# rust-seq/simd-minimizers

Hardware: AMD Instinct MI355X
Metric: Gbases/s (whole node) for canonical minimizers k=21 w=11 on 3.1 Gbp; HBM GB/s %peak (higher is better)
Workload: dtype u32

## Files before the change

### include/simd_minimizers_amd.h

```cpp
#ifndef SIMD_MINIMIZERS_AMD_H
#define SIMD_MINIMIZERS_AMD_H

#include <stddef.h>
#include <stdint.h>

#ifdef __cplusplus
extern "C" {
#endif


typedef struct mm_hasher {
    uint32_t fw[4];
    uint32_t rc[4];
    uint32_t rot;
    uint32_t canonical;
    uint32_t fw_xor;
    uint32_t rc_xor;
    uint32_t kind;
} mm_hasher_t;

typedef enum mm_hasher_kind { MM_HASHER_NT = 0, MM_HASHER_MUL = 1, MM_HASHER_ANTILEX = 2 } mm_hasher_kind_t;

typedef enum mm_mode { MM_MINIMIZERS = 0, MM_CLOSED_SYNCMERS = 1, MM_OPEN_SYNCMERS = 2 } mm_mode_t;

// ... 252 lines not shown

int mm_device_group_upload_batch(mm_device_group_t *group, uint64_t n_seqs, const uint8_t *const *packed,
                                 const uint64_t *packed_bytes);
int mm_run_batch_sharded_device(const mm_plan_t *plan, mm_device_group_t *group, const uint64_t *base_offsets ,
                                const uint64_t *n_bases, int want_superkmers, uint64_t *out_counts ,
                                uint64_t *total);
int mm_device_group_batch_result(const mm_device_group_t *group, uint64_t seq, int *entry, uint32_t **d_pos,
                                 uint32_t **d_sk, uint64_t *count);
int mm_device_group_gather_batch(mm_device_group_t *group, int root, uint32_t *d_dst_pos, uint32_t *d_dst_sk ,
                                 uint64_t capacity, uint64_t *out_offsets );

int mm_debug_launch_plan(uint32_t w, int canonical_windows, int mode, uint64_t n_seqs, const uint64_t *n_windows,
                         uint64_t *out7, uint32_t *tile_seq, uint32_t *tile_win0, uint32_t *tile_nblk,
                         uint64_t tile_capacity, uint64_t *n_tiles);
int mm_debug_launch_lds(uint32_t w, int canonical_windows, int mode, uint64_t n_windows, uint64_t *out2);
int mm_debug_lane_plan(uint32_t k, uint32_t w, int canonical_windows, int mode, uint64_t n_reads, uint64_t total_bases,
                       uint32_t blocks_per_lane, uint64_t *out6);
int mm_debug_last_lane_table(mm_workspace_t *ws, uint32_t *out4, uint64_t capacity, uint64_t *n_lanes);
int mm_link_probe(mm_workspace_t *ws, const void *host_in, void *host_out, uint64_t bytes, double *out_GBps );
int mm_clock_probe_begin(mm_workspace_t *ws, uint64_t duration_us);
int mm_clock_probe_end(mm_workspace_t *ws, double *ghz);
int mm_generate_device_async(mm_workspace_t *ws, uint64_t seed, uint64_t first_base,
                             uint64_t n_bases, uint8_t *d_packed );

#ifdef __cplusplus
}
#endif
#endif
```

### simd-minimizers_amd/__init__.py

```python
from __future__ import annotations

import ctypes as C
import os
import threading

import numpy as np

_HERE = os.path.dirname(os.path.abspath(__file__))
LIB_PATH = os.environ.get("MM_LIB_PATH") or os.path.join(_HERE, "libsimd_minimizers_amd.so")

MM_MINIMIZERS, MM_CLOSED_SYNCMERS, MM_OPEN_SYNCMERS = 0, 1, 2
PATH_FUSED, PATH_GENERIC, PATH_SPLIT = 1, 2, 3
U64_MAX = (1 << 64) - 1

ERR = {
    "W_ZERO": -1, "W_TOO_LARGE": -2, "LEN_TOO_LARGE": -3, "EVEN_L": -4,
    "HASHER_NOT_CANONICAL": -5, "OPEN_EVEN_W": -6, "K_ZERO": -7, "CAPACITY": -8, "BAD_MODE": -9,
    "NULL": -10, "VALUE_LEN": -11, "FORMAT": -12, "NO_DEVICE": -20, "HIP": -21, "ALLOC": -22, "ORDER": -23,
    "UNSORTED": -24,
}


class MinimizerError(RuntimeError):
    def __init__(self, code: int, msg: str):
# ... 118 lines not shown
            L.mm_device_group_upload_batch.argtypes = [vp, C.c_uint64, C.POINTER(u8p), u64p]
            L.mm_run_batch_sharded_device.argtypes = [vp, vp, u64p, u64p, C.c_int, u64p, u64p]
            L.mm_device_group_batch_result.argtypes = [vp, C.c_uint64, C.POINTER(C.c_int), C.POINTER(u32p), C.POINTER(u32p), u64p]
            L.mm_device_group_gather_batch.argtypes = [vp, C.c_int, vp, vp, C.c_uint64, u64p]
            L.mm_run_packed_reads_device_async.argtypes = [vp, vp, vp, C.c_uint64, C.c_uint64, C.c_uint64, vp, C.c_uint64,
                                                           C.c_uint32, vp, vp, C.c_uint64, vp, vp]
            L.mm_run_packed_reads_device.argtypes = [vp, vp, vp, C.c_uint64, C.c_uint64, C.c_uint64, vp, C.c_uint64,
                                                     C.c_uint32, vp, vp, C.c_uint64, vp, u64p]
            L.mm_run_packed_reads_host.argtypes = [vp, vp, u8p, C.c_uint64, u64p, C.c_uint32, u32p, u32p, C.c_uint64, u64p, u64p]
            L.mm_debug_launch_plan.argtypes = [C.c_uint32, C.c_int, C.c_int, C.c_uint64, u64p, u64p, u32p, u32p, u32p,
                                               C.c_uint64, u64p]
        L.mm_clock_probe_begin.argtypes = [vp, C.c_uint64]
        L.mm_clock_probe_end.argtypes = [vp, C.POINTER(C.c_double)]
        L.mm_link_probe.argtypes = [vp, vp, vp, C.c_uint64, C.POINTER(C.c_double)]
        L.mm_debug_launch_lds.argtypes = [C.c_uint32, C.c_int, C.c_int, C.c_uint64, u64p]
        L.mm_debug_lane_plan.argtypes = [C.c_uint32, C.c_uint32, C.c_int, C.c_int, C.c_uint64, C.c_uint64, C.c_uint32, u64p]
        L.mm_debug_last_lane_table.argtypes = [vp, u32p, C.c_uint64, u64p]
        L.mm_fused_overread_bytes.argtypes = []
        L.mm_fused_overread_bytes.restype = C.c_uint64
        L.mm_workspace_force_generic.argtypes = [vp, C.c_int]
        L.mm_workspace_set_blocks_per_lane.argtypes = [vp, C.c_uint32]
        L.mm_workspace_enable_timing.argtypes = [vp, C.c_int]
        L.mm_workspace_kernel_time.argtypes = [vp, C.POINTER(C.c_double), u64p, C.c_int]
        L.mm_workspace_last_path.argtypes = [vp]
        L.mm_workspace_ticket_mode.argtypes = [vp]
        L.mm_workspace_last_lane_table.argtypes = [vp]
        if hasattr(L, "mm_prebuilt_window_sizes"):
            L.mm_prebuilt_window_sizes.argtypes = [C.c_int, C.c_int, u32p, C.c_int]
            L.mm_prebuilt_window_sizes.restype = C.c_int
        L.mm_run_device_async.argtypes = [vp, vp, vp, C.c_uint64, C.c_uint64, C.c_uint64, C.c_uint64,
# ... 70 lines not shown
    "mm_run_device_async", "mm_run_device", "mm_run_host", "mm_run_host_ascii",
    "mm_values_u64_device_async", "mm_values_u64_host", "mm_values_u128_device_async",
    "mm_values_u128_host", "mm_run_batch_device", "mm_run_reads_device_async", "mm_run_reads_device",
    "mm_run_reads_superkmers_device_async", "mm_run_reads_superkmers_device",
    "mm_run_skip_ambiguous_device_async", "mm_run_skip_ambiguous_device", "mm_run_skip_ambiguous_host",
    "mm_run_skip_ambiguous_host_ascii", "mm_run_reads_skip_ambiguous_device_async",
    "mm_run_reads_skip_ambiguous_device", "mm_pack_ascii_n_device_async", "mm_pack_ascii_device_async",
    "mm_host_alloc", "mm_host_free",
    "mm_generate_device_async", "mm_fasta_pack_device_async", "mm_fasta_pack_device", "mm_fastq_pack_device_async",
    "mm_clock_probe_begin", "mm_clock_probe_end", "mm_link_probe", "mm_fused_overread_bytes",
    "mm_device_group_create", "mm_device_group_destroy", "mm_device_group_size", "mm_run_sharded_host",
    "mm_run_batch_sharded_host",
    "mm_device_group_upload", "mm_device_group_upload_range", "mm_device_group_adopt", "mm_run_sharded_device", "mm_device_group_result",
    "mm_device_group_gather",
    "mm_device_group_upload_batch", "mm_run_batch_sharded_device", "mm_device_group_batch_result",
    "mm_device_group_gather_batch", "mm_debug_launch_plan", "mm_debug_launch_lds", "mm_debug_lane_plan",
    "mm_debug_last_lane_table",
    "mm_run_packed_reads_device_async", "mm_run_packed_reads_device", "mm_run_packed_reads_host",
    "mm_text_mul_hasher", "mm_text_hasher_from_dna", "mm_plan_create_text", "mm_run_text_device_async",
    "mm_run_text_device", "mm_run_text_host", "mm_text_prebuilt_window_sizes",
    "mm_run_text_batch_device_async", "mm_run_text_batch_device", "mm_run_text_batch_host",
]


def prebuilt_window_sizes(canonical: bool, reads: bool = False) -> list:
    L = lib()
    n = L.mm_prebuilt_window_sizes(int(canonical), int(reads), None, 0)
    buf = (C.c_uint32 * max(1, n))()
    L.mm_prebuilt_window_sizes(int(canonical), int(reads), buf, n)
    return [int(x) for x in buf[:n]]

# ... 901 lines not shown
```

### simd-minimizers_amd/csrc/mm_api.hip

```cpp
#include <hip/hip_runtime.h>

#include <cstdio>
#include <cstdlib>
#include <chrono>
#include <cstring>
#include <new>
#include <algorithm>
#include <string>
#include <thread>
#include <utility>
#include <vector>

#include "../../include/simd_minimizers_amd.h"
#include "mm_env.h"
#include "mm_launch.h"

namespace {

struct ApiDeviceState {
    int depth = 0;
    int saved = -1;
    bool changed = false;
};
thread_local ApiDeviceState t_api_dev;
// ... 749 lines not shown
    a.scratch = nullptr;
    a.generic_round_windows = 0;
    a.timing_start = a.timing_stop = nullptr;
    return a;
}

int mm_debug_launch_lds(uint32_t w, int canonical_windows, int mode, uint64_t n_windows, uint64_t *out2) {
    ApiScope api_scope;
    if (!out2 || w == 0) return MM_ERR_NULL;
    const mm::RunArgs a = debug_plan_args(w, canonical_windows, mode, 0, n_windows);
    unsigned long long o[2];
    mm::fused_debug_lds(a, o);
    out2[0] = o[0];
    out2[1] = o[1];
    return MM_OK;
}

int mm_debug_launch_plan(uint32_t w, int canonical_windows, int mode, uint64_t n_seqs, const uint64_t *n_windows,
                         uint64_t *out7, uint32_t *tile_seq, uint32_t *tile_win0, uint32_t *tile_nblk, uint64_t tile_capacity,
                         uint64_t *n_tiles) {
    ApiScope api_scope;
    if (!n_windows || w == 0) return MM_ERR_NULL;
    mm::RunArgs a = debug_plan_args(w, canonical_windows, mode, n_seqs, n_windows[0]);
    if (n_seqs == 0) {
        if (!out7) return MM_ERR_NULL;
        unsigned long long o[7];
        mm::fused_debug_plan(a, o);
        for (int i = 0; i < 7; ++i) out7[i] = o[i];
        return MM_OK;
    }
// ... 3034 lines not shown
```

### simd-minimizers_amd/csrc/mm_fused.hip

```cpp
#include "mm_fused_impl.h"
#include "mm_fused_inst.h"
#include "mm_env.h"
#include "mm_launch.h"
#include "mm_split.h"

#include <cstdlib>
#include <cstdio>
#include <map>
#include <mutex>
#include <string>
#include <utility>
#include <vector>

namespace mm {

namespace {

using KernelFn = FusedKernelFn;
using Instance = FusedInstance;

uint32_t debug_switches() {
#ifdef MM_EXPERIMENTS
    const char *dbg = mm_exp_env("MM_DEBUG");
    return dbg ? (uint32_t)atoi(dbg) : 0u;
// ... 12 lines not shown
const Instance *find_instance(uint32_t w, int canonical_windows, int hasher_canonical) {
    using Getter = const Instance *(*)(int *);
    static const Getter kGroups[] = {fused_instances_a, fused_instances_b, fused_instances_c, fused_instances_d, fused_instances_e, fused_instances_f, fused_instances_g, fused_instances_h, fused_instances_i,
                                     fused_instances_j, fused_instances_k, fused_instances_l, fused_instances_m};
    for (Getter get : kGroups) {
        int n = 0;
        const Instance *inst = get(&n);
        for (int i = 0; i < n; ++i)
            if (inst[i].w == w && inst[i].canon == (canonical_windows != 0) &&
                inst[i].hash_rc == (hasher_canonical != 0))
                return &inst[i];
    }
    return nullptr;
}

double emit_density(uint32_t w, uint32_t mode) {
    return mode == 2 ? 1.0 / w : (mode == 1 ? 2.0 / w : 2.0 / (w + 1.0));
}

uint32_t list_capacity(uint32_t w, uint32_t mode, uint32_t S) {
    static const uint32_t extra = mm_exp_env("MM_CAP_EXTRA") ? (uint32_t)atoi(mm_exp_env("MM_CAP_EXTRA")) : 0u;
    uint32_t cap = (uint32_t)(1.3 * emit_density(w, mode) * S) + 8u + extra;
    return cap > S + w ? S + w : cap;
}

uint64_t status_stride_host() {
    static const uint64_t v = mm_exp_env("MM_STATUS_STRIDE_HOST") ? (uint64_t)atoi(mm_exp_env("MM_STATUS_STRIDE_HOST")) : kStatusStride;
    return v < kStatusStride ? kStatusStride : v;
}

// ... 72 lines not shown
    } else {
        const uint64_t nwin = a.win_end - a.win_begin;
        g.nblocks = (nwin + g.NB - 1) / g.NB;
    }
    return g;
}

struct KernelRef {
    KernelFn host = nullptr;
    hipFunction_t mod = nullptr;
    explicit operator bool() const { return host || mod; }
};

thread_local std::string t_jit_error;

KernelRef resolve_kernel(uint32_t w, int canonical_windows, int hasher_canonical, uint32_t mode, bool sk) {
    KernelRef kr;
    if (mode > 2) return kr;
    const bool force_jit = force_jit_wanted();
    const Instance *inst = force_jit ? nullptr : find_instance(w, canonical_windows, hasher_canonical);
    if (inst) {
        kr.host = inst->fn[(mode == 0 && sk) ? 3 : mode];
        return kr;
    }
    kr.mod = jit_fused_kernel(w, canonical_windows != 0, hasher_canonical != 0, (int)mode, mode == 0 && sk,
                              false, &t_jit_error);
    return kr;
}

int launch_kernel(const KernelRef &kr, uint32_t grid, uint32_t lds_bytes, hipStream_t stream, FusedParams &p,
                  hipEvent_t ev0, hipEvent_t ev1) {
    if (kr.host) {
        if (lds_bytes > 64u * 1024u &&
            hipFuncSetAttribute(reinterpret_cast<const void *>(kr.host),
// ... 26 lines not shown
        (void)hipGetLastError();
        t_jit_error = std::string("launch of the run-time specialised kernel rejected: ") + hipGetErrorString(e);
        return -2;
    }
    return 0;
}

}

const char *fused_unavailable_reason() { return t_jit_error.c_str(); }

bool fused_supported(uint32_t k, uint32_t w, int canonical_windows, int hasher_canonical) {
    (void)k;
    if (find_instance(w, canonical_windows, hasher_canonical)) return true;
    return jit_enabled() && w >= 1 && w <= kJitMaxW;
}

static uint32_t whole_rounds_lo(uint32_t nblk) { return nblk * 85u / 100u > 6u ? nblk * 85u / 100u : 6u; }

static uint64_t taper_extra_tiles() {
    int cus = 0, dev = 0;
    if (hipGetDevice(&dev) != hipSuccess ||
        hipDeviceGetAttribute(&cus, hipDeviceAttributeMultiprocessorCount, dev) != hipSuccess || cus < 1) {
        (void)hipGetLastError();
        cus = 512;
    }
    return 8ull * (uint64_t)cus + 64ull;
}

uint64_t fused_status_words(const RunArgs &a) {
// ... 100 lines not shown
    g.nblk = nb;
    g.S = a.w * g.nblk;
    g.list_cap = list_capacity(a.w, a.mode, g.S);
    g.lds_bytes = g.list_cap * stride_of(a);
    g.NB = kFusedThreads * g.S;
    g.nblocks = (nwin + g.NB - 1) / g.NB;
}

uint32_t fused_batch_nblk(const RunArgs &a, const uint64_t *n_windows, uint64_t n_seqs) {
    if (a.nblk != 0) return 0;
    Geometry g = geometry(a);
    uint64_t tiles = 0;
    for (uint64_t s = 0; s < n_seqs; ++s) tiles += (n_windows[s] + g.NB - 1) / g.NB;
    g.nblocks = tiles;
    if (tiles <= 512) return 0;
    const KernelRef kr = resolve_kernel(a.w, a.canonical_windows, (int)a.ht.canonical, a.mode, a.out.sk != nullptr);
    if (!kr) return 0;
    const uint32_t nb = whole_rounds_nblk(a, kr, g, [&](uint64_t S) {
        uint64_t t = 0;
        for (uint64_t s = 0; s < n_seqs; ++s) t += (n_windows[s] + kFusedThreads * S - 1) / (kFusedThreads * S);
        return t;
    });
    return nb == g.nblk ? 0u : nb;
}

constexpr uint32_t kTaperMinBlocksDefault = 4;
static uint32_t taper_min_blocks() {
    const char *e = mm_env("MM_TAPER_MIN_BLOCKS");
    const int v = e ? atoi(e) : 0;
    return v >= 1 ? (uint32_t)v : kTaperMinBlocksDefault;
}
// ... 40 lines not shown
    t.start = f1 * (uint64_t)g.NB;
    t.tiles = tiles;
    return t;
}

bool fused_batch_tiles(const RunArgs &a0, const uint64_t *n_windows, uint64_t n_seqs, std::vector<BatchTile> &tiles,
                       uint32_t *nblk_out) {
    RunArgs a = a0;
    Geometry g = geometry(a);
    uint64_t total = 0;
    for (uint64_t s = 0; s < n_seqs; ++s) total += n_windows[s];
    const uint64_t blk_w = (uint64_t)kFusedThreads * a.w;
    uint64_t zone_start = ~0ull, per_level = 1, lmax = 0;
    uint64_t fake_slots = 0;
    if (const char *e = mm_env("MM_TAPER_SLOTS")) fake_slots = (uint64_t)atoi(e) > 0 ? (uint64_t)atoi(e) : 0;
    const KernelRef kr = (a.nblk == 0 && total && !fake_slots) ? resolve_kernel(a.w, a.canonical_windows, (int)a.ht.canonical, a.mode, a.out.sk != nullptr) : KernelRef();
    int per_cu = 0, cus = 0;
    if (a.nblk == 0 && total && !mm_env("MM_NO_TAPER") && g.nblk >= kTaperMinBlocks + 4u &&
        (fake_slots || (kr && resident_slots(kr, g.lds_bytes, &per_cu, &cus)))) {
        const uint64_t slots = fake_slots ? fake_slots : (uint64_t)per_cu * cus;
        lmax = g.nblk - kTaperMinBlocks;
        per_level = (slots * taper_slots_pct() / 100 + lmax - 1) / lmax;
        const uint64_t cap_w = per_level * blk_w * (lmax * g.nblk - lmax * (lmax + 1) / 2);
        if (total >= cap_w + slots * (uint64_t)g.NB / 2) zone_start = total - cap_w;
    }
    if (zone_start == ~0ull && a.nblk == 0) {
        const uint32_t nb = fused_batch_nblk(a, n_windows, n_seqs);
        if (nb) {
            a.nblk = nb;
            g = geometry(a);
        }
// ... 53 lines not shown
    out[6] = (unsigned long long)kFusedThreads * a.w;
    return 0;
}

void fused_debug_lds(const RunArgs &a, unsigned long long *out2) {
    const Geometry g = geometry(a);
    out2[0] = g.lds_bytes;
    out2[1] = ambi_landing(a.w, a.wamb);
}

int launch_fused(const RunArgs &a, hipStream_t stream) {
    Geometry g = geometry(a);
    if (g.nblocks == 0) return 0;
    if (g.lds_bytes > kMaxLdsBytes) return -2;
    const KernelRef kr = resolve_kernel(a.w, a.canonical_windows, (int)a.ht.canonical, a.mode,
                                        a.out.sk != nullptr);
    if (!kr) return -2;
    const bool small_run = g.nblocks < 128 && !mm_env("MM_TAPER_SLOTS");
    if (!small_run && a.nblk == 0 && !a.batch_tile_seq && !mm_env("MM_NO_ONE_ROUND")) {
        RunArgs full = a;
        full.work_windows = 0;
        const Geometry gd = geometry(full);
        int per_cu = 0, cus = 0;
        uint64_t slots = 0;
        if (const char *e = mm_env("MM_TAPER_SLOTS")) slots = (uint64_t)atoi(e) > 0 ? (uint64_t)atoi(e) : 0;
        if (!slots && resident_slots(kr, gd.lds_bytes + ambi_landing(a.w, a.wamb), &per_cu, &cus)) slots = (uint64_t)per_cu * cus;
        if (slots) one_round_geometry(a, slots, gd, &g);
    }
    const bool tapers = !small_run && plan_taper(a, kr, g).first != 0xffffffffu && !mm_env("MM_TUNE_ALWAYS");
    if (!tapers && !small_run) {
        const Geometry untuned = g;
// ... 449 lines not shown
```

### simd-minimizers_amd/csrc/mm_fused_impl.h

```cpp
#pragma once
#include "mm_common.h"

#ifndef MM_LB_SLEEP_SHORT
#define MM_LB_SLEEP_SHORT 120
#endif
#ifndef MM_LB_SLEEP_CANON
#define MM_LB_SLEEP_CANON 32
#endif
#ifndef MM_STORE_MOD
#define MM_STORE_MOD "nt"
#endif
#ifndef MM_STORE_AUX
#define MM_STORE_AUX 2
#endif
#ifndef MM_PREFETCH_BLOCKS
#define MM_PREFETCH_BLOCKS 2
#endif
#ifdef MM_STAGE
#define MM_STAGE_GE(n) (MM_STAGE >= (n))
#else
#define MM_STAGE_GE(n) 1
#endif

#ifndef MM_STATUS_STRIDE
// ... 174 lines not shown
        }
        if (!ok) break;
    }
    return m;
}
constexpr int wide_dwords(int W) {
    const int m4 = wide_group_blocks_nd(W, 4), m5 = wide_group_blocks_nd(W, 5);
    return (m4 > 0 && 2 * m4 >= m5) ? 4 : 5;
}
constexpr int wide_group_blocks(int W) { return wide_group_blocks_nd(W, wide_dwords(W)); }
template <int W>
constexpr int kWideGroup = wide_group_blocks(W);
template <int W>
constexpr int kWideDwords = wide_dwords(W);

template <int N>
struct IntTag {
    static constexpr int value = N;
};

template <bool B>
struct BoolTag {
    static constexpr bool value = B;
};

struct LaneCtx {
    const uint2 *tab;
    long long p0;
    uint32_t lane_bases;
    uint32_t wbase;
// ... 14 lines not shown
constexpr uint32_t kLandQ4Bytes = 64u * 4u;
constexpr uint32_t amb_row_dwords(int W) { return W <= 37 ? 8u : (W <= 54 ? 11u : 16u); }
#ifndef MM_AMBI_LAND
#define MM_AMBI_LAND 1
#endif
#ifndef MM_AMBI_ROWS_MINW
#define MM_AMBI_ROWS_MINW 36
#endif
constexpr bool ambi_land_rule(int W) { return MM_AMBI_LAND && W >= 32 && W <= 96 && wide_group_blocks(W) != 0; }
constexpr bool ambi_rows_rule(int W) { return ambi_land_rule(W) && W >= MM_AMBI_ROWS_MINW; }
constexpr uint32_t land_amb_bytes(int W) { return ambi_rows_rule(W) ? amb_row_dwords(W) * 256u : 2u * 64u * 16u; }
constexpr uint32_t land_q4_bytes(int W) { return (ambi_rows_rule(W) ? 2u : 4u) * kLandQ4Bytes; }
constexpr uint32_t land_wave_bytes(int W) { return land_amb_bytes(W) + land_q4_bytes(W); }
constexpr uint32_t ambi_land_bytes(int W) { return ambi_land_rule(W) ? kFusedWaves * land_wave_bytes(W) : 0u; }

template <int W, bool CANON, bool HASH_RC, int MODE, bool SK, bool DIRECT, bool PARTIAL, bool AMBI = false, bool E8 = false>
__device__ __forceinline__ uint32_t lane_walk(const FusedParams &p, const LaneCtx &ctx, bool &overflowed) {
    static_assert(!E8 || !SK, "8-bit list entries hold positions only");
    constexpr uint32_t kStride = list_stride(E8);
    constexpr int NSUB = (W + 15) / 16;
    const uint32_t nblk = ctx.nblk;

    const long long P0 = ctx.p0;
    const long long Q0 = P0 >> 4;
    const long long Q0v = Q0 < 0 ? 0 : Q0;
    const long long Q0c =
        (long long)(((unsigned long long)(uint32_t)__builtin_amdgcn_readfirstlane((uint32_t)((unsigned long long)Q0v >> 32)) << 32) |
                    (unsigned long long)(uint32_t)__builtin_amdgcn_readfirstlane((uint32_t)Q0v));
    const int32_t prel0 = (int32_t)(P0 - (Q0c << 4));
    const __amdgpu_buffer_rsrc_t rsrc = __builtin_amdgcn_make_buffer_rsrc(
        const_cast<uint32_t *>(ctx.seq_d + Q0c), 0, (int)(((long long)ctx.seq_dwords - Q0c) * 4), 0x00020000);
// ... 10 lines not shown

    using RawView = decltype(__builtin_amdgcn_raw_buffer_load_b64(rsrc, 0, 0, 0));
    auto raw = [&](uint32_t pos) -> RawView {
#ifdef MM_EXP_LOADSAME
        return __builtin_amdgcn_raw_buffer_load_b64(rsrc, ((pos >> 4) << 2) & 0x78u, 0, 0);
#else
        return __builtin_amdgcn_raw_buffer_load_b64(rsrc, (pos >> 4) << 2, 0, 0);
#endif
    };
    auto aligned = [&](const RawView &d, uint32_t pos) -> uint32_t {
        return __builtin_amdgcn_alignbit(d[1], d[0], 2u * (pos & 15u));
    };

    const uint32_t rot_l = (32u - p.ht.rot) & 31u;
    const uint32_t rot_r = p.ht.rot & 31u;
    const uint32_t k = p.k;
    uint32_t fw = p.ht.fw0, rc = p.ht.rc0;
    const uint8_t *tabb = reinterpret_cast<const uint8_t *>(ctx.tab);

    const uint32_t rot2_l = (32u - 2u * p.ht.rot) & 31u, rot2_r = (2u * p.ht.rot) & 31u;
#ifdef MM_EXP_NOWARM
    for (uint32_t g = 0; g * 16u < 0u; ++g) {
#else
    for (uint32_t g = 0; g * 16u < k; ++g) {
#endif
        const uint32_t wa = g == 0 ? view_first(pb) : view(pb + 16u * g);
        const uint32_t rem = k - 16u * g;
#pragma unroll
        for (int m = 0; m < 8; ++m) {
            if ((uint32_t)(2 * m + 1) < rem) {
                const uint32_t a8 = (m == 0 ? (wa << 3) : (wa >> (4 * m - 3))) & 0x78u;
// ... 67 lines not shown
    auto land_q4_load = [&](uint32_t gpos, uint32_t par, uint32_t which) {
        const uint32_t off = (gpos >> 4) << 2;
        const uint32_t base = __builtin_amdgcn_readfirstlane(land + q4_off(par, which));
        __builtin_amdgcn_raw_ptr_buffer_load_lds(rsrc, (LdsPtr)(uintptr_t)base, 4, off, 16, 0, 0);
    };
    auto land_q4_read = [&](uint32_t par, uint32_t which) -> uint32_t {
        return lds_u32(land + q4_off(par, which) + 4u * lane_id_now());
    };
    auto wide_normalise = [&](WideBuf &dst, const WideBuf &w) -> uint32_t {
        const uint32_t a = w.sh >> 3;
#pragma unroll
        for (int i = 0; i < ND; ++i)
            dst.q[i] = __builtin_amdgcn_alignbyte(i + 1 < ND ? w.q[i + 1 < ND ? i + 1 : i] : 0u, w.q[i], a);
        return w.sh & 6u;
    };
    auto wide_views = [&](const WideBuf &w, uint32_t sh, auto ktag, uint32_t (&v)[NSUB]) {
        constexpr int K = decltype(ktag)::value;
#pragma unroll
        for (int g = 0; g < NSUB; ++g) {
            const int p = (2 * W * K + 32 * g) / 32;
            v[g] = __builtin_amdgcn_alignbit(p + 1 < ND ? w.q[p + 1 < ND ? p + 1 : 0] : 0u, w.q[p < ND ? p : 0], sh);
        }
    };
#pragma unroll
    for (int g = 0; g < NSUB; ++g) {
        va[g] = view(pos_in + 16u * (uint32_t)g);
        vr[g] = g == 0 ? view_first(pos_out) : view(pos_out + 16u * (uint32_t)g);
        v2[g] = 0;
    }

// ... 21 lines not shown
        }
        if (MG == 0) {
#pragma unroll
            for (int d = 0; d < PFD - 1; ++d)
#pragma unroll
                for (int g = 0; g < NSUB; ++g) {
                    qa[d][g] = raw(pos_in + (uint32_t)((d + 1) * W + 16 * g));
                    qr[d][g] = raw(pos_out + (uint32_t)((d + 1) * W + 16 * g));
                    if (kV2Load) q2[d][g] = raw(pb + 1u + (uint32_t)((d + 1) * W + 16 * g));
                }
        } else {
            gp_in = pos_in + (uint32_t)W;
            gp_out = pos_out + (uint32_t)W;
            wide_load(gp_in, Wa[1]);
#ifndef MM_EXP_ONE_STREAM
            wide_load(gp_out, Wr[1]);
#endif
            if (kAmbiLand && ND == 5) {
                land_q4_load(gp_in, lpar, 0u);
                land_q4_load(gp_out, lpar, 1u);
            }
            gp_in += (uint32_t)(MG * W);
            gp_out += (uint32_t)(MG * W);
        }
#pragma unroll
        for (int j = 0; j < W; ++j) {
            const uint32_t h = HASH_RC ? fw + rc : fw;
            const uint32_t kl = (h & kmask) | (uint32_t)j;
            ring_l[j] = kl;
            if (CANON) ring_r[j] = kl ^ kmask;
            const int jj = j & 15, g = j >> 4, m = jj >> 1;
            const uint32_t mw = (jj & 1) ? mo[g] : me[g];
// ... 154 lines not shown
#else
                tgw[g] = (((x ^ y) >> 1) & 0x55555555u) | ((y & ~x) & 0xAAAAAAAAu);
#endif
                } else {
                const int kCnt = (W - 16 * g) >= 16 ? 16 : (W - 16 * g);
                const uint32_t kBlockMask = 0xAAAAAAAAu & (kCnt >= 16 ? 0xffffffffu : ((1u << (2 * (kCnt > 0 ? kCnt : 0))) - 1u));
                xt[g] = x & kBlockMask;
                yt[g] = y & kBlockMask;
                }
            }
        }
        pos_in += W;
        pos_out += W;
        pos_r2 += W;
        MM_BUMP(sh_in, 2 * W);
        MM_BUMP(sh_out, 2 * W);
        if (MG == 0) {
            MM_BUMP(pl_in, W);
            MM_BUMP(pl_out, W);
        }
        if (CANON && !kV2Load) {
            uint32_t t2[NSUB];
#pragma unroll
            for (int g = 0; g < NSUB; ++g) t2[g] = next_base_view(vr, g);
#pragma unroll
            for (int g = 0; g < NSUB; ++g) {
                v2[g] = t2[g];
                asm volatile("" : "+v"(v2[g]));
            }
        }
        if (AMBI && kAmbiLand) {
// ... 13 lines not shown
            if (kAmbRows) {
                if (ka + 1u == kAmbChunkBlocks) {
                    asm volatile("s_waitcnt lgkmcnt(0)" ::: "memory");
                    land_rows_load(ctx.abase + b * (uint32_t)W);
                    ka = 0u;
                } else {
                    ka += 1u;
                }
            } else {
                apar ^= 1u;
                land_amb_load(ctx.abase + b * (uint32_t)W, apar);
            }
        }
        if (MG != 0) {
            if ((KN >= 0 ? (uint32_t)KN : kn) == 0u) {
                sh_in = wide_normalise(Wa[0], Wa[1]);
#ifdef MM_EXP_ONE_STREAM
                sh_out = sh_in;
                wide_load(gp_in, Wa[1]);
                MM_BUMP(gp_in, MG * W);
#else
                sh_out = wide_normalise(Wr[0], Wr[1]);
                wide_load(gp_in, Wa[1]);
                wide_load(gp_out, Wr[1]);
                if (kAmbiLand && ND == 5) {
                    if (kQ4One) asm volatile("s_waitcnt lgkmcnt(0)" ::: "memory");
                    land_q4_load(gp_in, lpar, 0u);
                    land_q4_load(gp_out, lpar, 1u);
                }
                MM_BUMP(gp_in, MG * W);
                MM_BUMP(gp_out, MG * W);
#endif
            }
            switch (KN >= 0 ? (uint32_t)KN : kn) {
#define MM_WIDE_CASE(K)                                                   \
    case K:                                                               \
        if (K < (MG ? MG : 1)) {                                          \
            wide_views(Wa[0], sh_in, IntTag<(K < (MG ? MG : 1) ? K : 0)>{}, va); \
            wide_views(Wr[0], sh_out, IntTag<(K < (MG ? MG : 1) ? K : 0)>{}, vr); \
        }                                                                 \
        break;
                MM_WIDE_CASE(0)
                MM_WIDE_CASE(1)
                MM_WIDE_CASE(2)
                MM_WIDE_CASE(3)
                MM_WIDE_CASE(4)
                MM_WIDE_CASE(5)
                MM_WIDE_CASE(6)
                MM_WIDE_CASE(7)
#undef MM_WIDE_CASE
                default: break;
            }
            if (KN < 0) kn = (kn + 1 == (uint32_t)(MG ? MG : 1)) ? 0u : kn + 1u;
        } else
// ... 633 lines not shown
                for (uint32_t c = (uint32_t)kWave + lane; c < n; c += kWave) {
                    const uint8_t *q = rd + kEB * L + (c - lane) * kStride;
                    const uint32_t e1 = E8 ? (uint32_t)*q : (uint32_t)*reinterpret_cast<const uint16_t *>(q);
                    const uint32_t iw = e1 >> kSh;
                    __builtin_amdgcn_raw_buffer_store_b32(SK ? vb + iw + (e1 & kRelMask) : vb + e1, opos,
                                                          (off + c) * 4u, 0, 0);
                    if (SK) __builtin_amdgcn_raw_buffer_store_b32(vb + 1u + iw, osk, (off + c) * 4u, 0, 0);
                }
            }
        }
        }
    }
    }
}

template <int W, bool CANON, bool HASH_RC, int MODE, bool SK, bool READS>
#ifndef MM_MIN_BLOCKS
#define MM_MIN_BLOCKS                                                                                             \
    (!CANON && !READS && !SK && W <= 13                                                                           \
         ? 7                                                                                                      \
         : (W <= 12 ? 4                                                                                           \
                    : (CANON && !READS ? (W >= 19 && W <= 37 ? 4 : (W >= 38 && W <= 54 ? 3 : (W >= 55 && W <= 64 ? 2 : 1))) \
                                       : 1)))
#endif
#ifndef MM_MIN_BLOCKS_WALK
#define MM_MIN_BLOCKS_WALK MM_MIN_BLOCKS
#endif
__global__ __launch_bounds__(kFusedThreads, MM_MIN_BLOCKS) void fused_kernel(const FusedParams p) {
    extern __shared__ __attribute__((aligned(16))) uint8_t smem[];
    __shared__ uint2 s_tab[36];
    __shared__ uint32_t s_bid;
// ... 211 lines not shown
        ctx.lane_bases = lw;
        ctx.wbase = (uint32_t)bw0 + lw;
        ctx.no_prev = (bw0 + lw == 0);
        ctx.rem_valid = (int)nvalid - (int)lw;
        ctx.abase = (uint32_t)bw0 + lw;
        set_min_rem(lane_active);
        if (redo) {
            my_count = reinterpret_cast<const uint16_t *>(p.dump + (size_t)bid * p.dump_stride)[tid];
        } else if (const bool dirty = (kAmbi && p.wamb) ? wave_has_skipped(p, ctx, S, lane_active) : false;
                   lane_active && !(MM_DBG(p) & 4u)) {
            bool over = false;
            if (kAmbi && p.wamb && dirty)
                my_count = (partial || !kTwoBodies<W>)
                               ? lane_walk<W, CANON, HASH_RC, MODE, SK, false, true, kAmbi, kE8>(p, ctx, over)
                               : lane_walk<W, CANON, HASH_RC, MODE, SK, false, kAmbi && !kTwoBodies<W>, kAmbi, kE8>(p, ctx, over);
            else my_count = partial ? lane_walk<W, CANON, HASH_RC, MODE, SK, false, true, false, kE8>(p, ctx, over)
                                    : lane_walk<W, CANON, HASH_RC, MODE, SK, false, false, false, kE8>(p, ctx, over);
            if (over) s_overflow = 1;
        }
    }

#ifdef MM_PRIO_P2
    __builtin_amdgcn_s_setprio(MM_PRIO_P2);
#endif
    if (p.trace && tid == 0) p.trace[10 * (size_t)bid + 1] = wall_clock64();
    const uint32_t incl = wave_scan_dpp(my_count);
    const uint32_t wave_total = __builtin_amdgcn_readlane(incl, kWave - 1);
    if (lane == 0) {
        s_wave_tot[wave] = wave_total;
        if (atomicAdd(&s_done, 1u) == (uint32_t)(kFusedWaves - 1) && bid != 0 && !(MM_DBG(p) & 1u) && !redo) {
            uint32_t tot = 0;
#pragma unroll
// ... 45 lines not shown
        unsigned long long o = run0 + excl;
        for (uint32_t j = 0; j < R; ++j) {
            const bool act = setup_read(j);
            ctx.dst = o;
            bool over;
            if (act) {
                if (kAmbi && p.wamb) lane_walk<W, CANON, HASH_RC, MODE, SK, true, true, kAmbi, kE8>(p, ctx, over);
                else lane_walk<W, CANON, HASH_RC, MODE, SK, true, true, false, kE8>(p, ctx, over);
            }
            o += (read_counts >> (16u * j)) & 0xffffu;
        }
    } else if (lane_active) {
        ctx.dst = run0 + excl;
        bool over;
        if (kAmbi && p.wamb) lane_walk<W, CANON, HASH_RC, MODE, SK, true, true, kAmbi, kE8>(p, ctx, over);
        else if (partial) lane_walk<W, CANON, HASH_RC, MODE, SK, true, true, false, kE8>(p, ctx, over);
        else lane_walk<W, CANON, HASH_RC, MODE, SK, true, false, false, kE8>(p, ctx, over);
    }
    if (p.trace) {
        __syncthreads();
        if (tid == 0) p.trace[10 * (size_t)bid + 3] = wall_clock64();
    }
    if (tid == 0 && bid == gridDim.x - 1 && !redo) {
        *p.out.total = s_excl + block_total;
        if (p.out.count_out) *p.out.count_out = s_excl + block_total;
        if (p.out.total_host)
            __hip_atomic_store(p.out.total_host, s_excl + block_total, __ATOMIC_RELAXED, __HIP_MEMORY_SCOPE_SYSTEM);
        if (READS) p.read_offsets[p.n_reads] = s_excl + block_total;
        if (batch) p.batch_offsets[p.batch_n] = s_excl + block_total;
    }
}

// ... 119 lines not shown
```

### simd-minimizers_amd/csrc/mm_fused_inst.h

```cpp
#pragma once
#include "mm_fused_impl.h"

namespace mm {

using FusedKernelFn = void (*)(const FusedParams);

struct FusedInstance {
    uint32_t w;
    bool canon;
    bool hash_rc;
    FusedKernelFn fn[4];
};

#define MM_FUSED_INST(W, C, R)                                                              \
    {                                                                                       \
        W, C, R, {                                                                          \
            &fused_kernel<W, C, R, 0, false, false>, &fused_kernel<W, C, R, 1, false, false>, \
                &fused_kernel<W, C, R, 2, false, false>, &fused_kernel<W, C, R, 0, true, false> \
        }                                                                                   \
    }

const FusedInstance *fused_instances_a(int *count);
const FusedInstance *fused_instances_b(int *count);
const FusedInstance *fused_instances_c(int *count);
const FusedInstance *fused_instances_d(int *count);
const FusedInstance *fused_instances_e(int *count);
const FusedInstance *fused_instances_f(int *count);
const FusedInstance *fused_instances_g(int *count);
const FusedInstance *fused_instances_h(int *count);
const FusedInstance *fused_instances_i(int *count);
const FusedInstance *fused_instances_j(int *count);
const FusedInstance *fused_instances_k(int *count);
const FusedInstance *fused_instances_l(int *count);
const FusedInstance *fused_instances_m(int *count);

struct FusedReadsInstance {
    uint32_t w;
    bool canon;
    bool hash_rc;
    FusedKernelFn fn;
};
#define MM_READS_INST(W, C, R) \
    { W, C, R, &fused_kernel<W, C, R, 0, false, true> }
const FusedReadsInstance *fused_reads_instances_a(int *count);
const FusedReadsInstance *fused_reads_instances_b(int *count);
const FusedReadsInstance *fused_reads_instances_c(int *count);
const FusedReadsInstance *fused_reads_instances_d(int *count);
const FusedReadsInstance *fused_reads_instances_e(int *count);

struct WalkInstance {
// ... 12 lines not shown
```

### simd-minimizers_amd/csrc/mm_launch.h

```cpp
#pragma once
#include <hip/hip_runtime.h>
#include <stdint.h>

#include <string>
#include <vector>

#include "mm_common.h"

namespace mm {

struct RunArgs {
    SeqView seq;
    HashTables ht;
    uint32_t k, w;
    int canonical_windows;
    uint32_t mode;
    uint64_t win_begin, win_end;
    OutParams out;
    const uint32_t *wamb;
    uint32_t wamb_dwords;
    const BatchSeq *batch_seqs;
    const BatchTile *batch_tile_seq;
    unsigned long long *batch_offsets;
    uint32_t batch_n;
// ... 1 lines not shown
    uint32_t nblk;
    uint64_t work_windows;
    int use_ticket;
    uint64_t status_avail = 0;
    uint32_t status_epoch = 0;
    bool append = false;
    void *scratch;
    uint64_t generic_round_windows;
    hipEvent_t timing_start, timing_stop;
};

constexpr uint32_t kFusedMaxLaneWindows = 60000u;
uint64_t fused_overread_bytes();

bool fused_supported(uint32_t k, uint32_t w, int canonical_windows, int hasher_canonical);
uint64_t fused_status_words(const RunArgs &a);
uint64_t fused_status_stride();
uint32_t fused_tile_windows(const RunArgs &a);
uint32_t fused_batch_nblk(const RunArgs &a, const uint64_t *n_windows, uint64_t n_seqs);
int fused_debug_plan(const RunArgs &a, unsigned long long *out );
void fused_debug_lds(const RunArgs &a, unsigned long long *out2);
bool fused_batch_tiles(const RunArgs &a, const uint64_t *n_windows, uint64_t n_seqs, std::vector<BatchTile> &tiles,
                       uint32_t *nblk_out);
int launch_fused(const RunArgs &a, hipStream_t stream);
const char *fused_unavailable_reason();
int fused_prebuilt_windows(bool canonical, bool reads, uint32_t *out, int capacity);

struct SplitBuffers {
    uint8_t *dump = nullptr;
    uint64_t dump_bytes = 0;
// ... 131 lines not shown
```

Baseline: 2053.

## Add fixed-k fused kernel instance that derives outgoing bases from the incoming stream

```diff
diff --git a/include/simd_minimizers_amd.h b/include/simd_minimizers_amd.h
--- a/include/simd_minimizers_amd.h
+++ b/include/simd_minimizers_amd.h
@@ -290,6 +290,7 @@
                          uint64_t *out7, uint32_t *tile_seq, uint32_t *tile_win0, uint32_t *tile_nblk,
                          uint64_t tile_capacity, uint64_t *n_tiles);
 int mm_debug_launch_lds(uint32_t w, int canonical_windows, int mode, uint64_t n_windows, uint64_t *out2);
+int mm_debug_fixed_k_kernel(uint32_t k, uint32_t w, int canonical_windows);
 int mm_debug_lane_plan(uint32_t k, uint32_t w, int canonical_windows, int mode, uint64_t n_reads, uint64_t total_bases,
                        uint32_t blocks_per_lane, uint64_t *out6);
 int mm_debug_last_lane_table(mm_workspace_t *ws, uint32_t *out4, uint64_t capacity, uint64_t *n_lanes);
diff --git a/simd-minimizers_amd/__init__.py b/simd-minimizers_amd/__init__.py
--- a/simd-minimizers_amd/__init__.py
+++ b/simd-minimizers_amd/__init__.py
@@ -156,6 +156,7 @@
         L.mm_clock_probe_end.argtypes = [vp, C.POINTER(C.c_double)]
         L.mm_link_probe.argtypes = [vp, vp, vp, C.c_uint64, C.POINTER(C.c_double)]
         L.mm_debug_launch_lds.argtypes = [C.c_uint32, C.c_int, C.c_int, C.c_uint64, u64p]
+        L.mm_debug_fixed_k_kernel.argtypes = [C.c_uint32, C.c_uint32, C.c_int]
         L.mm_debug_lane_plan.argtypes = [C.c_uint32, C.c_uint32, C.c_int, C.c_int, C.c_uint64, C.c_uint64, C.c_uint32, u64p]
         L.mm_debug_last_lane_table.argtypes = [vp, u32p, C.c_uint64, u64p]
         L.mm_fused_overread_bytes.argtypes = []
@@ -256,7 +257,7 @@
     "mm_device_group_upload", "mm_device_group_upload_range", "mm_device_group_adopt", "mm_run_sharded_device", "mm_device_group_result",
     "mm_device_group_gather",
     "mm_device_group_upload_batch", "mm_run_batch_sharded_device", "mm_device_group_batch_result",
-    "mm_device_group_gather_batch", "mm_debug_launch_plan", "mm_debug_launch_lds", "mm_debug_lane_plan",
+    "mm_device_group_gather_batch", "mm_debug_launch_plan", "mm_debug_launch_lds", "mm_debug_lane_plan", "mm_debug_fixed_k_kernel",
     "mm_debug_last_lane_table",
     "mm_run_packed_reads_device_async", "mm_run_packed_reads_device", "mm_run_packed_reads_host",
     "mm_text_mul_hasher", "mm_text_hasher_from_dna", "mm_plan_create_text", "mm_run_text_device_async",
diff --git a/simd-minimizers_amd/csrc/mm_api.hip b/simd-minimizers_amd/csrc/mm_api.hip
--- a/simd-minimizers_amd/csrc/mm_api.hip
+++ b/simd-minimizers_amd/csrc/mm_api.hip
@@ -787,6 +787,10 @@
     out2[0] = o[0];
     out2[1] = o[1];
     return MM_OK;
+}
+
+int mm_debug_fixed_k_kernel(uint32_t k, uint32_t w, int canonical_windows) {
+    return mm::fused_fixed_k(k, w, canonical_windows, canonical_windows) ? 1 : 0;
 }
 
 int mm_debug_launch_plan(uint32_t w, int canonical_windows, int mode, uint64_t n_seqs, const uint64_t *n_windows,
diff --git a/simd-minimizers_amd/csrc/mm_fused.hip b/simd-minimizers_amd/csrc/mm_fused.hip
--- a/simd-minimizers_amd/csrc/mm_fused.hip
+++ b/simd-minimizers_amd/csrc/mm_fused.hip
@@ -50,6 +50,17 @@
     return nullptr;
 }
 
+const FusedKcInstance *find_kc_instance(uint32_t w, uint32_t k, int canonical_windows, int hasher_canonical) {
+    if (mm_exp_env("MM_NO_KC")) return nullptr;
+    int n = 0;
+    const FusedKcInstance *inst = fused_kc_instances(&n);
+    for (int i = 0; i < n; ++i)
+        if (inst[i].w == w && inst[i].k == k && inst[i].canon == (canonical_windows != 0) &&
+            inst[i].hash_rc == (hasher_canonical != 0))
+            return &inst[i];
+    return nullptr;
+}
+
 double emit_density(uint32_t w, uint32_t mode) {
     return mode == 2 ? 1.0 / w : (mode == 1 ? 2.0 / w : 2.0 / (w + 1.0));
 }
@@ -152,10 +163,16 @@
 
 thread_local std::string t_jit_error;
 
-KernelRef resolve_kernel(uint32_t w, int canonical_windows, int hasher_canonical, uint32_t mode, bool sk) {
+KernelRef resolve_kernel(uint32_t w, int canonical_windows, int hasher_canonical, uint32_t mode, bool sk, uint32_t k = 0) {
     KernelRef kr;
     if (mode > 2) return kr;
     const bool force_jit = force_jit_wanted();
+    if (k != 0 && mode == 0 && !sk && !force_jit) {
+        if (const FusedKcInstance *kc = find_kc_instance(w, k, canonical_windows, hasher_canonical)) {
+            kr.host = kc->fn;
+            return kr;
+        }
+    }
     const Instance *inst = force_jit ? nullptr : find_instance(w, canonical_windows, hasher_canonical);
     if (inst) {
         kr.host = inst->fn[(mode == 0 && sk) ? 3 : mode];
@@ -212,6 +229,10 @@
     (void)k;
     if (find_instance(w, canonical_windows, hasher_canonical)) return true;
     return jit_enabled() && w >= 1 && w <= kJitMaxW;
+}
+
+bool fused_fixed_k(uint32_t k, uint32_t w, int canonical_windows, int hasher_canonical) {
+    return !force_jit_wanted() && find_kc_instance(w, k, canonical_windows, hasher_canonical) != nullptr;
 }
 
 static uint32_t whole_rounds_lo(uint32_t nblk) { return nblk * 85u / 100u > 6u ? nblk * 85u / 100u : 6u; }
@@ -342,7 +363,7 @@
     for (uint64_t s = 0; s < n_seqs; ++s) tiles += (n_windows[s] + g.NB - 1) / g.NB;
     g.nblocks = tiles;
     if (tiles <= 512) return 0;
-    const KernelRef kr = resolve_kernel(a.w, a.canonical_windows, (int)a.ht.canonical, a.mode, a.out.sk != nullptr);
+    const KernelRef kr = resolve_kernel(a.w, a.canonical_windows, (int)a.ht.canonical, a.mode, a.out.sk != nullptr, a.k);
     if (!kr) return 0;
     const uint32_t nb = whole_rounds_nblk(a, kr, g, [&](uint64_t S) {
         uint64_t t = 0;
@@ -413,7 +434,7 @@
     uint64_t zone_start = ~0ull, per_level = 1, lmax = 0;
     uint64_t fake_slots = 0;
     if (const char *e = mm_env("MM_TAPER_SLOTS")) fake_slots = (uint64_t)atoi(e) > 0 ? (uint64_t)atoi(e) : 0;
-    const KernelRef kr = (a.nblk == 0 && total && !fake_slots) ? resolve_kernel(a.w, a.canonical_windows, (int)a.ht.canonical, a.mode, a.out.sk != nullptr) : KernelRef();
+    const KernelRef kr = (a.nblk == 0 && total && !fake_slots) ? resolve_kernel(a.w, a.canonical_windows, (int)a.ht.canonical, a.mode, a.out.sk != nullptr, a.k) : KernelRef();
     int per_cu = 0, cus = 0;
     if (a.nblk == 0 && total && !mm_env("MM_NO_TAPER") && g.nblk >= kTaperMinBlocks + 4u &&
         (fake_slots || (kr && resident_slots(kr, g.lds_bytes, &per_cu, &cus)))) {
@@ -497,7 +518,7 @@
     if (g.nblocks == 0) return 0;
     if (g.lds_bytes > kMaxLdsBytes) return -2;
     const KernelRef kr = resolve_kernel(a.w, a.canonical_windows, (int)a.ht.canonical, a.mode,
-                                        a.out.sk != nullptr);
+                                        a.out.sk != nullptr, a.k);
     if (!kr) return -2;
     const bool small_run = g.nblocks < 128 && !mm_env("MM_TAPER_SLOTS");
     if (!small_run && a.nblk == 0 && !a.batch_tile_seq && !mm_env("MM_NO_ONE_ROUND")) {
diff --git a/simd-minimizers_amd/csrc/mm_fused_impl.h b/simd-minimizers_amd/csrc/mm_fused_impl.h
--- a/simd-minimizers_amd/csrc/mm_fused_impl.h
+++ b/simd-minimizers_amd/csrc/mm_fused_impl.h
@@ -212,6 +212,26 @@
 template <int W>
 constexpr int kWideDwords = wide_dwords(W);
 
+constexpr bool kc_rule(int W, int KC) {
+#ifdef MM_NO_KC
+    return false;
+#endif
+    if (KC <= 0) return false;
+    const int MG = wide_group_blocks(W), ND = wide_dwords(W);
+    if (MG < 1 || (MG * W) % 4 != 0) return false;
+    if ((KC + 2 * W - 1) / 4 - MG * W / 4 < -4) return false;
+    const int nsub = (W + 15) / 16, valid = 32 * ND - 24, span = 2 * MG * W;
+    for (int K = 0; K < MG; ++K)
+        for (int g = 0; g < nsub; ++g) {
+            int off = 2 * W * K + 32 * g - 2 * KC;
+            if (off < 0) off += span;
+            if (off < 0) return false;
+            const int bases = (W - 16 * g < 16 ? W - 16 * g : 16) + (g == nsub - 1 ? 1 : 0);
+            if (off % 32 > 24 || off + 6 + 2 * bases > valid) return false;
+        }
+    return true;
+}
+
 template <int N>
 struct IntTag {
     static constexpr int value = N;
@@ -256,7 +276,7 @@
 constexpr uint32_t land_wave_bytes(int W) { return land_amb_bytes(W) + land_q4_bytes(W); }
 constexpr uint32_t ambi_land_bytes(int W) { return ambi_land_rule(W) ? kFusedWaves * land_wave_bytes(W) : 0u; }
 
-template <int W, bool CANON, bool HASH_RC, int MODE, bool SK, bool DIRECT, bool PARTIAL, bool AMBI = false, bool E8 = false>
+template <int W, bool CANON, bool HASH_RC, int MODE, bool SK, bool DIRECT, bool PARTIAL, bool AMBI = false, bool E8 = false, int KC = 0>
 __device__ __forceinline__ uint32_t lane_walk(const FusedParams &p, const LaneCtx &ctx, bool &overflowed) {
     static_assert(!E8 || !SK, "8-bit list entries hold positions only");
     constexpr uint32_t kStride = list_stride(E8);
@@ -297,7 +317,8 @@
 
     const uint32_t rot_l = (32u - p.ht.rot) & 31u;
     const uint32_t rot_r = p.ht.rot & 31u;
-    const uint32_t k = p.k;
+    constexpr bool kKC = !AMBI && kc_rule(W, KC);
+    const uint32_t k = kKC ? (uint32_t)KC : p.k;
     uint32_t fw = p.ht.fw0, rc = p.ht.rc0;
     const uint8_t *tabb = reinterpret_cast<const uint8_t *>(ctx.tab);
 
@@ -395,6 +416,21 @@
             dst.q[i] = __builtin_amdgcn_alignbyte(i + 1 < ND ? w.q[i + 1 < ND ? i + 1 : i] : 0u, w.q[i], a);
         return w.sh & 6u;
     };
+    auto kc_out_views = [&](const WideBuf &wp, const WideBuf &w, uint32_t sh, auto ktag, uint32_t (&v)[NSUB]) {
+        constexpr int K = decltype(ktag)::value;
+        constexpr int kSpan = 2 * W * (MG ? MG : 1);
+#pragma unroll
+        for (int g = 0; g < NSUB; ++g) {
+            constexpr int kLag = 2 * (KC > 0 ? KC : 0);
+            const int off0 = 2 * W * K + 32 * g - kLag;
+            const bool prv = off0 < 0;
+            const int off = prv ? off0 + kSpan : off0;
+            const int pp = off > 0 ? off / 32 : 0;
+            const uint32_t add = (uint32_t)(((off - 2 * W * K) % 32 + 32) % 32);
+            const WideBuf &src = prv ? wp : w;
+            v[g] = __builtin_amdgcn_alignbit(pp + 1 < ND ? src.q[pp + 1 < ND ? pp + 1 : 0] : 0u, src.q[pp < ND ? pp : 0], sh + add);
+        }
+    };
     auto wide_views = [&](const WideBuf &w, uint32_t sh, auto ktag, uint32_t (&v)[NSUB]) {
         constexpr int K = decltype(ktag)::value;
 #pragma unroll
@@ -446,8 +482,20 @@
             gp_out = pos_out + (uint32_t)W;
             wide_load(gp_in, Wa[1]);
 #ifndef MM_EXP_ONE_STREAM
-            wide_load(gp_out, Wr[1]);
-#endif
+            if (!kKC) wide_load(gp_out, Wr[1]);
+#endif
+            if (kKC) {
+                const int32_t A = (int32_t)(gp_in >> 2) - (MG * W) / 4;
+                const bool before = A < 0;
+                const uint32_t off = before ? 0u : ((uint32_t)A & ~3u);
+                typedef uint32_t u32x4w __attribute__((ext_vector_type(4)));
+                const u32x4w v = __builtin_amdgcn_raw_buffer_load_b128(rsrc, off, 0, 0);
+                const uint32_t v4 = ND == 5 ? __builtin_amdgcn_raw_buffer_load_b32(rsrc, off, 16, 0) : 0u;
+                const uint32_t x[6] = {before ? 0u : v.x, before ? v.x : v.y, before ? v.y : v.z, before ? v.z : v.w,
+                                       before ? v.w : v4, 0u};
+#pragma unroll
+                for (int i = 0; i < ND; ++i) Wa[0].q[i] = __builtin_amdgcn_alignbyte(i + 1 < ND ? x[i + 1] : 0u, x[i], (uint32_t)A & 3u);
+            }
             if (kAmbiLand && ND == 5) {
                 land_q4_load(gp_in, lpar, 0u);
                 land_q4_load(gp_out, lpar, 1u);
@@ -632,7 +680,7 @@
         pos_out += W;
         pos_r2 += W;
         MM_BUMP(sh_in, 2 * W);
-        MM_BUMP(sh_out, 2 * W);
+        if (!kKC) MM_BUMP(sh_out, 2 * W);
         if (MG == 0) {
             MM_BUMP(pl_in, W);
             MM_BUMP(pl_out, W);
@@ -676,7 +724,15 @@
         }
         if (MG != 0) {
             if ((KN >= 0 ? (uint32_t)KN : kn) == 0u) {
+                if (kKC) {
+#pragma unroll
+                    for (int i = 0; i < ND; ++i) Wr[0].q[i] = Wa[0].q[i];
+                }
                 sh_in = wide_normalise(Wa[0], Wa[1]);
+                if (kKC) {
+                    wide_load(gp_in, Wa[1]);
+                    MM_BUMP(gp_in, MG * W);
+                } else {
 #ifdef MM_EXP_ONE_STREAM
                 sh_out = sh_in;
                 wide_load(gp_in, Wa[1]);
@@ -693,13 +749,15 @@
                 MM_BUMP(gp_in, MG * W);
                 MM_BUMP(gp_out, MG * W);
 #endif
+                }
             }
             switch (KN >= 0 ? (uint32_t)KN : kn) {
 #define MM_WIDE_CASE(K)                                                   \
     case K:                                                               \
         if (K < (MG ? MG : 1)) {                                          \
             wide_views(Wa[0], sh_in, IntTag<(K < (MG ? MG : 1) ? K : 0)>{}, va); \
-            wide_views(Wr[0], sh_out, IntTag<(K < (MG ? MG : 1) ? K : 0)>{}, vr); \
+            if (kKC) kc_out_views(Wr[0], Wa[0], sh_in, IntTag<(K < (MG ? MG : 1) ? K : 0)>{}, vr); \
+            else wide_views(Wr[0], sh_out, IntTag<(K < (MG ? MG : 1) ? K : 0)>{}, vr); \
         }                                                                 \
         break;
                 MM_WIDE_CASE(0)
@@ -1363,7 +1421,7 @@
     }
 }
 
-template <int W, bool CANON, bool HASH_RC, int MODE, bool SK, bool READS>
+template <int W, bool CANON, bool HASH_RC, int MODE, bool SK, bool READS, int KC = 0>
 #ifndef MM_MIN_BLOCKS
 #define MM_MIN_BLOCKS                                                                                             \
     (!CANON && !READS && !SK && W <= 13                                                                           \
@@ -1605,8 +1663,8 @@
                 my_count = (partial || !kTwoBodies<W>)
                                ? lane_walk<W, CANON, HASH_RC, MODE, SK, false, true, kAmbi, kE8>(p, ctx, over)
                                : lane_walk<W, CANON, HASH_RC, MODE, SK, false, kAmbi && !kTwoBodies<W>, kAmbi, kE8>(p, ctx, over);
-            else my_count = partial ? lane_walk<W, CANON, HASH_RC, MODE, SK, false, true, false, kE8>(p, ctx, over)
-                                    : lane_walk<W, CANON, HASH_RC, MODE, SK, false, false, false, kE8>(p, ctx, over);
+            else my_count = partial ? lane_walk<W, CANON, HASH_RC, MODE, SK, false, true, false, kE8, KC>(p, ctx, over)
+                                    : lane_walk<W, CANON, HASH_RC, MODE, SK, false, false, false, kE8, KC>(p, ctx, over);
             if (over) s_overflow = 1;
         }
     }
@@ -1682,8 +1740,8 @@
         ctx.dst = run0 + excl;
         bool over;
         if (kAmbi && p.wamb) lane_walk<W, CANON, HASH_RC, MODE, SK, true, true, kAmbi, kE8>(p, ctx, over);
-        else if (partial) lane_walk<W, CANON, HASH_RC, MODE, SK, true, true, false, kE8>(p, ctx, over);
-        else lane_walk<W, CANON, HASH_RC, MODE, SK, true, false, false, kE8>(p, ctx, over);
+        else if (partial) lane_walk<W, CANON, HASH_RC, MODE, SK, true, true, false, kE8, KC>(p, ctx, over);
+        else lane_walk<W, CANON, HASH_RC, MODE, SK, true, false, false, kE8, KC>(p, ctx, over);
     }
     if (p.trace) {
         __syncthreads();
diff --git a/simd-minimizers_amd/csrc/mm_fused_inst.h b/simd-minimizers_amd/csrc/mm_fused_inst.h
--- a/simd-minimizers_amd/csrc/mm_fused_inst.h
+++ b/simd-minimizers_amd/csrc/mm_fused_inst.h
@@ -34,6 +34,15 @@
 const FusedInstance *fused_instances_l(int *count);
 const FusedInstance *fused_instances_m(int *count);
 
+struct FusedKcInstance {
+    uint32_t w, k;
+    bool canon, hash_rc;
+    FusedKernelFn fn;
+};
+#define MM_KC_INST(W, KC, C, R) \
+    { W, KC, C, R, &fused_kernel<W, C, R, 0, false, false, KC> }
+const FusedKcInstance *fused_kc_instances(int *count);
+
 struct FusedReadsInstance {
     uint32_t w;
     bool canon;
diff --git a/simd-minimizers_amd/csrc/mm_fused_inst_kc.hip b/simd-minimizers_amd/csrc/mm_fused_inst_kc.hip
--- /dev/null
+++ b/simd-minimizers_amd/csrc/mm_fused_inst_kc.hip
@@ -0,0 +1,27 @@
+#include "mm_fused_impl.h"
+#include "mm_fused_inst.h"
+
+namespace mm {
+
+#ifndef MM_NO_KC
+static_assert(kc_rule(11, 21), "k=21 w=11 walks with one load stream");
+static_assert(!kc_rule(51, 31), "k=31 w=51: listed here once the rule admits it");
+#endif
+
+const FusedKcInstance *fused_kc_instances(int *count) {
+#ifndef MM_NO_KC
+    static const FusedKcInstance kInst[] = {
+        MM_KC_INST(11, 21, true, true),
+#ifdef MM_KC_FORWARD
+        MM_KC_INST(11, 21, false, false),
+#endif
+    };
+    *count = (int)(sizeof(kInst) / sizeof(kInst[0]));
+    return kInst;
+#else
+    *count = 0;
+    return nullptr;
+#endif
+}
+
+}
diff --git a/simd-minimizers_amd/csrc/mm_launch.h b/simd-minimizers_amd/csrc/mm_launch.h
--- a/simd-minimizers_amd/csrc/mm_launch.h
+++ b/simd-minimizers_amd/csrc/mm_launch.h
@@ -39,6 +39,7 @@
 uint64_t fused_overread_bytes();
 
 bool fused_supported(uint32_t k, uint32_t w, int canonical_windows, int hasher_canonical);
+bool fused_fixed_k(uint32_t k, uint32_t w, int canonical_windows, int hasher_canonical);
 uint64_t fused_status_words(const RunArgs &a);
 uint64_t fused_status_stride();
 uint32_t fused_tile_windows(const RunArgs &a);
```

Measured after the change: 2104, median of 6. +2.5%, better.
